# divyanshu-kumar/openh264-wasm

Hardware: AMD Instinct MI355X
Metric: 1080p30 frames/sec encode+decode per GPU (parity vs oracle; OpenH264 parity unpinned) (higher is better)
Workload: dtype u8

## Files before the change

### openh264-wasm_amd/csrc/dec_recon.inc

```
namespace h264mi {

struct DecLaunch { int S, mbw, mbh; const DecDesc *desc; uint32_t *ticket; const DbkDesc *dbk; uint64_t *prof; uint32_t tag; int streamed; };

struct DecGateLaunch { int S; const DecDesc *desc; uint32_t tag; uint32_t rows; };
__global__ __launch_bounds__(64) void dec_gate_kernel(DecGateLaunch a) {
    for (int s = 0; s < a.S; s++) {
        const DecDesc &D = a.desc[s];
        if (!D.st->got_pic) continue;
        GLOBAL uint64_t *prog = gbl(&D.frm->prog);
        WaitClock wc;
        for (unsigned spins = 0; ((spins & 255) != 255) || !wc.expired(); spins++) {
            uint64_t x = 0;
            if (threadIdx.x == 0) x = __hip_atomic_load(prog, __ATOMIC_RELAXED, __HIP_MEMORY_SCOPE_AGENT);
            const uint32_t t = (uint32_t)__builtin_amdgcn_readfirstlane((int)(uint32_t)(x >> 32));
            const uint32_t v = (uint32_t)__builtin_amdgcn_readfirstlane((int)(uint32_t)x);
            if (t == a.tag && v >= a.rows) break;
            __builtin_amdgcn_s_sleep(8);
        }
    }
}

struct DecWaitLaunch { const uint32_t *counter; uint32_t target; uint32_t limit_ticks; };
__global__ __launch_bounds__(64) void dec_wait_counter_kernel(DecWaitLaunch a) {
    const uint64_t t0 = __builtin_amdgcn_s_memrealtime();
// ... 12 lines not shown
    for (unsigned spins = 0;; spins++) {
        uint64_t x = 0;
        if (threadIdx.x == 0) x = __hip_atomic_load(prog, __ATOMIC_RELAXED, __HIP_MEMORY_SCOPE_AGENT);
        const uint32_t t = (uint32_t)__builtin_amdgcn_readfirstlane((int)(uint32_t)(x >> 32));
        const uint32_t v = (uint32_t)__builtin_amdgcn_readfirstlane((int)(uint32_t)x);
        if (t == tag) {
            if (v == H264MI_PROG_ABORT) break;
            if (v >= need) {
                __builtin_amdgcn_fence(__ATOMIC_ACQUIRE, "agent");
                asm volatile("s_waitcnt vmcnt(0)" ::: "memory");
                return true;
            }
        }
        if ((spins & 255) == 255) {
            const int ab = __hip_atomic_load(abort_word, __ATOMIC_RELAXED, __HIP_MEMORY_SCOPE_AGENT);
            if (ab || wc.expired()) break;
        }
        __builtin_amdgcn_s_sleep(2);
    }
    if (threadIdx.x == 0) __hip_atomic_store(abort_word, 1, __ATOMIC_RELAXED, __HIP_MEMORY_SCOPE_AGENT);
    return false;
}

#ifndef H264MI_REC_TILE
#define H264MI_REC_TILE 0
#endif
struct DecLds {
    alignas(16) uint8_t win[4][64 * 64];
    alignas(16) uint8_t winc[2][32 * 32];
    alignas(16) uint32_t cf[208];
#if H264MI_REC_TILE
    alignas(16) uint8_t tile[48 * 48];
#endif
    alignas(16) int16_t res[24][16];
    int dcval[24];
    alignas(16) uint8_t rec[256];
    alignas(16) uint8_t recc[2][64];
#if H264MI_REC_TILE
    alignas(16) uint8_t pcm[384];
#endif
    uint8_t top[24];
    uint8_t topc[2][12];
    uint8_t left[16], leftc[2][8];
    uint8_t n4[16];
    uint32_t gp[3][8];
    uint32_t gm[3][5];
    int8_t modes[16];
    alignas(16) MbInfo info;
    alignas(16) MbInfo linfo;
};

DEV uint32_t dwin4(const DecLds &S, int p, int wr, int gx) {
    const int sl = (gx + 24) & 63;
    const uint32_t *row = (const uint32_t *)&S.win[p][wr * WIN_RING];
    return __builtin_amdgcn_alignbyte(row[((sl >> 2) + 1) & 15], row[sl >> 2], sl & 3);
}

struct TileGet {
    const uint8_t *t; int x0, y0;
    DEV int operator()(int x, int y) const { return t[(y - y0) * 48 + (x - x0)]; }
};
struct GlobGet {
    GLOBAL const uint8_t *p; int w, h;
    DEV int operator()(int x, int y) const { return p[clip3(0, h - 1, y) * w + clip3(0, w - 1, x)]; }
};
template <class G> DEV int g_b1(const G &g, int x, int y) { return tap6(g(x - 2, y), g(x - 1, y), g(x, y), g(x + 1, y), g(x + 2, y), g(x + 3, y)); }
template <class G> DEV int g_b(const G &g, int x, int y) { return clip1((g_b1(g, x, y) + 16) >> 5); }
template <class G> DEV int g_h(const G &g, int x, int y) {
    return clip1((tap6(g(x, y - 2), g(x, y - 1), g(x, y), g(x, y + 1), g(x, y + 2), g(x, y + 3)) + 16) >> 5);
}
template <class G> DEV int g_j(const G &g, int x, int y) {
    return clip1((tap6(g_b1(g, x, y - 2), g_b1(g, x, y - 1), g_b1(g, x, y), g_b1(g, x, y + 1), g_b1(g, x, y + 2), g_b1(g, x, y + 3)) + 512) >> 10);
}
template <class G> DEV int qpel(const G &g, int x, int y, int fx, int fy) {
    switch (fy * 4 + fx) {
    case 0: return g(x, y);
    case 1: return AVG(g(x, y), g_b(g, x, y));
    case 2: return g_b(g, x, y);
    case 3: return AVG(g_b(g, x, y), g(x + 1, y));
    case 4: return AVG(g(x, y), g_h(g, x, y));
    case 5: return AVG(g_b(g, x, y), g_h(g, x, y));
    case 6: return AVG(g_b(g, x, y), g_j(g, x, y));
    case 7: return AVG(g_b(g, x, y), g_h(g, x + 1, y));
    case 8: return g_h(g, x, y);
// ... 148 lines not shown
                    const int dx = I.mv[ras][0], dy = I.mv[ras][1];
                    int mx, my;
                    rmvp(S, mbx, nbm, done, px, py, sw, 0, mx, my);
                    set_part_mv(I, done, px, py, sw, sh, mx + dx, my + dy);
                }
        }
    } else if (type == MI_I4) {
        for (int blk = 0; blk < 16; blk++) S.modes[blk] = I.i4mode[blk];
        const uint32_t top = S.gm[mbx % 3][4] >> 8;
        for (int blk = 0; blk < 16; blk++) {
            const int ras = BLK2RAS[blk], x4 = ras & 3, y4 = ras >> 2;
            const int ma = x4 > 0 ? I.i4mode[ras - 1] : ((nbm & NB_A) ? S.linfo.i4mode[ras + 3] : -1);
            const int mb = y4 > 0 ? I.i4mode[ras - 4] : ((nbm & NB_B) ? (int)((top >> (4 * x4)) & 15) : -1);
            const int pm = (ma < 0 || mb < 0) ? 2 : min(ma, mb);
            const int code = (uint8_t)S.modes[blk];
            I.i4mode[ras] = (int8_t)(code == 0xff ? pm : (code < pm ? code : code + 1));
        }
    }
}

DEV bool mb_in_window(const MbInfo &I) {
    const int b = threadIdx.x & 15;
    const uint32_t mv = ((const uint32_t *)I.mv)[b];
    const int x = (b & 3) * 4 + ((int)(int16_t)(mv & 0xffff) >> 2), y = (b >> 2) * 4 + ((int)(int16_t)(mv >> 16) >> 2);
    const bool ok = min(x, y) >= -24 && max(x, y) + 5 <= 40;
    return __ballot(!ok) == 0;
}

#ifdef H264MI_REC_WPE
#define H264MI_REC_WPE_ATTR __attribute__((amdgpu_waves_per_eu(H264MI_REC_WPE, H264MI_REC_WPE)))
#else
#define H264MI_REC_WPE_ATTR
#endif
__global__ __launch_bounds__(64) H264MI_REC_WPE_ATTR void dec_recon_kernel(DecLaunch a) {
    __shared__ union { DecLds r; DbkLds d; } SH;
    DecLds &S = SH.r;
    __shared__ int s_ticket;
#ifndef H264MI_REC_RELANE
#define H264MI_REC_RELANE 1
#endif
#if H264MI_REC_RELANE
#define lane (e_tid() & 63)
#else
    const int lane = threadIdx.x;
#endif
    if (lane == 0) s_ticket = (int)atomicAdd(a.ticket, 1u);
    wave_lds_sync();
    const int t = uni(s_ticket), nrows = a.S * a.mbh;
    if (t >= nrows) {
// ... 3 lines not shown
        if (DD.active && uni(*DD.active) == 0) return;
        const DbkLaunch dl{a.mbw, a.mbh, a.S, a.dbk, nullptr, nullptr};
        deblock_row(SH.d, dl, DD, dby, DbkSrcGranules{gbl((const uint64_t *)DD.src_gran), a.mbw, dby, (uint32_t)uni((int)*DD.epoch)});
        return;
    }
    const int mby = t / a.S, sidx = t % a.S;
    CONSTANT const DecDesc &D = cst(a.desc)[sidx];
    DecState *st = D.st;
    if (!uni(st->got_pic)) return;
    const uint32_t epoch = (uint32_t)uni((int)st->epoch);
    const int par = uni(st->parity) & 1;
    const bool has_ref = uni(st->has_ref) != 0;
    const Xf XF = xf_consts(lane & 15);
    GLOBAL const uint8_t *R0 = gbl(D.pic[par][0]), *R1 = gbl(D.pic[par][1]), *R2 = gbl(D.pic[par][2]);
    GLOBAL uint32_t *info32 = gbl((uint32_t *)D.info);
    GLOBAL const MbCoef *coefg = gbl((const MbCoef *)D.coef);
    GLOBAL uint64_t *egr = gbl(D.egran);
    int32_t *abort_word = &st->err;
    if (a.streamed && !prog_wait(gbl(&D.frm->prog), a.tag, (uint32_t)mby + 1, abort_word)) return;
    const int mbw = a.mbw, cw = mbw * 16, ch = a.mbh * 16, ccw = cw / 2, cch = ch / 2;
    const int Y = mby * 16;
    GLOBAL uint64_t *grow_prev = gbl(D.gran) + (size_t)(mby > 0 ? mby - 1 : 0) * mbw * H264MI_GRANULES_PER_MB;
    GLOBAL uint64_t *grow = gbl(D.gran) + (size_t)mby * mbw * H264MI_GRANULES_PER_MB;
    const int Y0 = Y - 24;
    GLOBAL const uint8_t *plw[4];
    for (int k = 0; k < 4; k++) plw[k] = gbl((const uint8_t *)D.pl[k]) + (ptrdiff_t)(Y0 + lane) * D.ps;
    GLOBAL const uint8_t *plcw = gbl((const uint8_t *)D.plc[lane >> 5]) + (ptrdiff_t)(mby * 8 - 12 + (lane & 31)) * D.psc;
    uint32_t pf_info = 0, pf_cf[4] = {0, 0, 0, 0};
    u32x4 pf_w[4];
    u32x2 pf_c = {0, 0};
    auto issue = [&](int mx) {
        const int mi = mby * mbw + mx;
        if (lane < 32) pf_info = info32[(size_t)mi * 32 + lane];
        GLOBAL const uint32_t *cf32 = (GLOBAL const uint32_t *)(coefg + mi);
#pragma unroll
        for (int k = 0; k < 4; k++) if (lane + 64 * k < 208) pf_cf[k] = cf32[lane + 64 * k];
        if (has_ref && mx > 0) {
#pragma unroll
            for (int k = 0; k < 4; k++) pf_w[k] = *(GLOBAL const u32x4 *)(plw[k] + 16 * mx + 24);
            pf_c = *(GLOBAL const u32x2 *)(plcw + 8 * mx + 12);
        }
    };
    if (has_ref) {
#pragma unroll
        for (int k = 0; k < 4; k++)
#pragma unroll
            for (int j = 0; j < 4; j++) *(u32x4 *)&S.win[k][lane * WIN_RING + 16 * j] = *(GLOBAL const u32x4 *)(plw[k] - 24 + 16 * j);
#pragma unroll
        for (int j = 0; j < 4; j++) *(u32x2 *)&S.winc[lane >> 5][(lane & 31) * WINC_RING + 8 * j] = *(GLOBAL const u32x2 *)(plcw - 12 + 8 * j);
    }
    issue(0);
    uint64_t t_prev = a.prof ? clock64() : 0, s_prof[9] = {0, 0, 0, 0, 0, 0, 0, 0, 0};
    auto lap = [&](int k) { if (a.prof) { const uint64_t tt = clock64(); s_prof[k] += tt - t_prev; t_prev = tt; } };

    int pix_next = 0;
    for (int mbx = 0; mbx < mbw; mbx++) {
        const int X = mbx * 16, mbi = mby * mbw + mbx;
        if (lane < 32) ((uint32_t *)&S.info)[lane] = pf_info;
        const uint32_t rw0 = __builtin_amdgcn_readfirstlane(pf_info), rw31 = __builtin_amdgcn_readlane(pf_info, 31);
        const int rt = (int)(rw0 & 255);
        {
            if (rt == MI_I16 || rt == MI_IPCM || ((rw0 >> 16) & 255) != 0) {
#pragma unroll
                for (int k = 0; k < 4; k++) if (lane + 64 * k < 208) S.cf[lane + 64 * k] = pf_cf[k];
            }
        }
        if (mbx + 1 < mbw) issue(mbx + 1);
        lap(1);
        if (mby > 0) {
            uint32_t v;
// ... 21 lines not shown
        const uint32_t nbm = uni(mb_nb_mask(mbx, mby, mbw, MB_SLICE_FIRST(rw31)));
        if (rt == MI_PSKIP || rt == MI_P16x16) {
            const uint32_t mvw = resolve_p16_uni(S, mbx, nbm, rt == MI_PSKIP);
            if (lane >= 8 && lane < 13)
                gran_store(grow + (size_t)mbx * H264MI_GRANULES_PER_MB + lane, epoch, lane < 12 ? mvw : (uint32_t)rt | 0x222200u);
            wave_lds_sync();
        } else {
            if (lane == 0) resolve_record(S, mbx, nbm);
            wave_lds_sync();
        }
        if (lane >= 8 && lane < 13 && !(rt == MI_PSKIP || rt == MI_P16x16)) {
            const MbInfo &R = S.info;
            const uint32_t v = lane < 12 ? ((const uint32_t *)R.mv)[12 + lane - 8]
                                         : (uint32_t)R.type | ((uint32_t)(R.i4mode[12] & 15) << 8) | ((uint32_t)(R.i4mode[13] & 15) << 12) |
                                               ((uint32_t)(R.i4mode[14] & 15) << 16) | ((uint32_t)(R.i4mode[15] & 15) << 20);
            gran_store(grow + (size_t)mbx * H264MI_GRANULES_PER_MB + lane, epoch, v);
        }
        if (lane < 32) gran_store(egr + (size_t)mbi * 128 + 96 + lane, epoch, ((const uint32_t *)&S.info)[lane]);
        const MbInfo &I = S.info;
        const int type = I.type;
        const bool intra = type == MI_I4 || type == MI_I16, ipcm = type == MI_IPCM;
        lap(3);
        const MbCoef &CF = *(const MbCoef *)S.cf;
#if H264MI_REC_TILE
        if (ipcm) for (int k = lane; k < 384; k += 64) S.pcm[k] = ((const uint8_t *)&CF)[k];
        const uint8_t *PCM = S.pcm;
#else
        const uint8_t *PCM = (const uint8_t *)&CF;
#endif
        const bool has_top = nbm & NB_B, has_left = nbm & NB_A, has_tr = nbm & NB_C, has_tl = nbm & NB_D;
        const uint32_t *PB = S.gp[mbx % 3], *PC = S.gp[(mbx + 1) % 3], *PD = S.gp[(mbx + 2) % 3];
        if (intra) {
        if (lane < 21) {
            int v = 0;
            if (lane == 0) v = has_tl ? (PD[3] >> 24) & 255 : 0;
            else if (lane <= 16) v = has_top ? (PB[(lane - 1) >> 2] >> (8 * ((lane - 1) & 3))) & 255 : 0;
            else v = has_tr ? (PC[(lane - 17) >> 2] >> (8 * ((lane - 17) & 3))) & 255 : 0;
            S.top[lane] = (uint8_t)v;
        }
        if (lane >= 32 && lane < 50) {
            int pl = (lane - 32) / 9, k = (lane - 32) % 9, v = 0;
            if (k == 0) v = has_tl ? (PD[5 + 2 * pl] >> 24) & 255 : 0;
            else v = has_top ? (PB[4 + 2 * pl + ((k - 1) >> 2)] >> (8 * ((k - 1) & 3))) & 255 : 0;
            S.topc[pl][k] = (uint8_t)v;
        }
        if (!has_left && lane < 16) { S.left[lane] = 0; S.leftc[lane >> 3][lane & 7] = 0; }
        }
        wave_lds_sync();
        lap(4);
        const bool has_res = type != MI_PSKIP && !ipcm;
        if (has_res) {
            const QuantQP ql = make_qqp(I.qp), qcc = make_qqp(I.qpc);
// ... 50 lines not shown
                    }
                    S.n4[lane] = (uint8_t)v;
                }
                wave_lds_sync();
                if (lane < 16) {
                    const int m = I.i4mode[ras];
                    int s4t = S.n4[1] + S.n4[2] + S.n4[3] + S.n4[4], s4l = S.n4[9] + S.n4[10] + S.n4[11] + S.n4[12];
                    int dcv = (bt && bl) ? (s4t + s4l + 4) >> 3 : bl ? (s4l + 2) >> 2 : bt ? (s4t + 2) >> 2 : 128;
                    int pv = m == 2 ? dcv : i4_tap_eval(c_I4.t[m][lane], S.n4);
                    S.rec[(oy + (lane >> 2)) * 16 + ox + (lane & 3)] = (uint8_t)clip1(pv + S.res[ras][lane]);
                }
                wave_lds_sync();
            }
        } else if (type == MI_I16) {
            const I16Ctx k16 = i16_ctx(S, has_top, has_left);
            for (int i = lane; i < 256; i += 64) {
                int x = i & 15, y = i >> 4, ras = (y >> 2) * 4 + (x >> 2);
                S.rec[i] = (uint8_t)clip1(i16_pred(S, k16, I.i16mode, x, y) + S.res[ras][(y & 3) * 4 + (x & 3)]);
            }
        } else if (inwin) {
            {
                const int y = lane >> 2, x0 = (lane & 3) * 4, ras = (y >> 2) * 4 + (x0 >> 2);
                const int mx = I.mv[ras][0], my = I.mv[ras][1];
                const QSel q = qsel((my & 3) * 4 + (mx & 3));
                const int gx = X + x0 + (mx >> 2), wr = Y + y + (my >> 2) - Y0;
                const uint32_t pa = dwin4(S, q.p1, wr + q.dy1, gx + q.dx1), pb = dwin4(S, q.p2, wr + q.dy2, gx + q.dx2);
                const uint32_t pv = (pa | pb) - (((pa ^ pb) & 0xFEFEFEFEu) >> 1);
                uint32_t o = 0;
                if (has_res) {
                    const u32x2 r2 = *(const u32x2 *)&S.res[ras][(y & 3) * 4];
#pragma unroll
                    for (int j = 0; j < 4; j++) {
                        const int rj = (int16_t)(((j < 2 ? r2.x : r2.y) >> (16 * (j & 1))) & 0xffff);
                        o |= (uint32_t)clip1((int)((pv >> (8 * j)) & 255) + rj) << (8 * j);
                    }
                } else o = pv;
                *(uint32_t *)&S.rec[y * 16 + x0] = o;
            }
        } else {
#if H264MI_REC_TILE
            int x0 = 1 << 30, y0 = 1 << 30, x1 = -(1 << 30), y1 = -(1 << 30);
            for (int b = 0; b < 16; b++) {
                int ix = X + (b & 3) * 4 + (I.mv[b][0] >> 2), iy = Y + (b >> 2) * 4 + (I.mv[b][1] >> 2);
                x0 = min(x0, ix - 2); y0 = min(y0, iy - 2); x1 = max(x1, ix + 4 + 3); y1 = max(y1, iy + 4 + 3);
            }
            const bool use_tile = (x1 - x0) <= 48 && (y1 - y0) <= 48;
            if (use_tile) {
                for (int i = lane; i < 48 * 48; i += 64) {
                    int tx = i % 48, ty = i / 48;
                    S.tile[i] = R0[clip3(0, ch - 1, y0 + ty) * cw + clip3(0, cw - 1, x0 + tx)];
                }
                wave_lds_sync();
            }
            const TileGet tg{S.tile, x0, y0};
#endif
            const GlobGet gg{R0, cw, ch};
            for (int i = lane; i < 256; i += 64) {
                int x = i & 15, y = i >> 4, ras = (y >> 2) * 4 + (x >> 2);
                int mx = I.mv[ras][0], my = I.mv[ras][1];
                int gx = X + x + (mx >> 2), gy = Y + y + (my >> 2);
#if H264MI_REC_TILE
                int pv = use_tile ? qpel(tg, gx, gy, mx & 3, my & 3) : qpel(gg, gx, gy, mx & 3, my & 3);
#else
                int pv = qpel(gg, gx, gy, mx & 3, my & 3);
#endif
                S.rec[i] = (uint8_t)clip1(pv + (has_res ? S.res[ras][(y & 3) * 4 + (x & 3)] : 0));
            }
        }
        lap(6);
        if (!ipcm) {
            if (intra) {
                const CCtx kc = chroma_ctx(S, has_top, has_left);
                for (int i = lane; i < 128; i += 64) {
                    int pl = i >> 6, p = i & 63, x = p & 7, y = p >> 3;
                    int dv = chroma_dc_blk(S, kc, pl, x >> 2, y >> 2);
                    int pv = chroma_pred(S, kc, I.cmode, pl, x, y, dv);
                    S.recc[pl][p] = (uint8_t)clip1(pv + S.res[16 + 4 * pl + (y >> 2) * 2 + (x >> 2)][(y & 3) * 4 + (x & 3)]);
                }
            } else if (inwin) {
                const int p = lane, x = p & 7, y = p >> 3, ras = (y >> 1) * 4 + (x >> 1);
                const int mx = I.mv[ras][0], my = I.mv[ras][1], fx = mx & 7, fy = my & 7;
                const int cx = mbx * 8 + x + (mx >> 3), r0 = (y + (my >> 3) + 12) * WINC_RING, r1 = r0 + WINC_RING;
                const int c0 = (cx + 12) & 31, c1 = (cx + 13) & 31;
                const int w00 = (8 - fx) * (8 - fy), w01 = fx * (8 - fy), w10 = (8 - fx) * fy, w11 = fx * fy;
                const int rb = (y >> 2) * 2 + (x >> 2), ri = (y & 3) * 4 + (x & 3);
                int pv[2], rs[2];
#pragma unroll
                for (int pl = 0; pl < 2; pl++) {
// ... 9 lines not shown
                    int ras = (y >> 1) * 4 + (x >> 1);
                    int mx = I.mv[ras][0], my = I.mv[ras][1];
                    int fx = mx & 7, fy = my & 7, gx = mbx * 8 + x + (mx >> 3), gy = mby * 8 + y + (my >> 3);
                    GLOBAL const uint8_t *Rp = pl ? R2 : R1;
                    int xa = clip3(0, ccw - 1, gx), xb = clip3(0, ccw - 1, gx + 1), ya = clip3(0, cch - 1, gy), yb = clip3(0, cch - 1, gy + 1);
                    int A = Rp[ya * ccw + xa], B = Rp[ya * ccw + xb], C = Rp[yb * ccw + xa], E = Rp[yb * ccw + xb];
                    int pv = ((8 - fx) * (8 - fy) * A + fx * (8 - fy) * B + (8 - fx) * fy * C + fx * fy * E + 32) >> 6;
                    S.recc[pl][p] = (uint8_t)clip1(pv + (has_res ? S.res[16 + 4 * pl + (y >> 2) * 2 + (x >> 2)][(y & 3) * 4 + (x & 3)] : 0));
                }
            }
        }
        wave_lds_sync();
        lap(7);
        gran_store(egr + (size_t)mbi * 128 + lane, epoch, ((const uint32_t *)S.rec)[lane]);
        if (lane < 32) gran_store(egr + (size_t)mbi * 128 + 64 + lane, epoch, ((const uint32_t *)S.recc[lane >> 4])[((lane >> 1) & 7) * 2 + (lane & 1)]);
        if (lane < 8) {
            const uint32_t v = lane < 4 ? ((const uint32_t *)S.rec)[60 + lane] : ((const uint32_t *)S.recc[(lane - 4) >> 1])[14 + (lane & 1)];
            gran_store(grow + (size_t)mbx * H264MI_GRANULES_PER_MB + lane, epoch, v);
        }
        if (lane < 16) { S.left[lane] = S.rec[lane * 16 + 15]; S.leftc[lane >> 3][lane & 7] = S.recc[lane >> 3][(lane & 7) * 8 + 7]; }
        if (lane < 32) ((uint32_t *)&S.linfo)[lane] = ((const uint32_t *)&S.info)[lane];
        if (has_ref && mbx + 1 < mbw) {
            const int nx = mbx + 1;
#pragma unroll
            for (int k = 0; k < 4; k++) *(u32x4 *)&S.win[k][lane * WIN_RING + ((16 * nx + 48) & 63)] = pf_w[k];
            *(u32x2 *)&S.winc[lane >> 5][(lane & 31) * WINC_RING + ((8 * nx + 24) & 31)] = pf_c;
        }
        wave_lds_sync();
        lap(8);
    }
    if (a.prof && lane == 0) {
#pragma unroll
        for (int k = 1; k < 9; k++) atomicAdd((unsigned long long *)&a.prof[k], (unsigned long long)s_prof[k]);
    }
#if H264MI_REC_RELANE
#undef lane
#endif
}

struct DecEndLaunch { int S; const DecDesc *desc; int check; };
__global__ void dec_end_kernel(DecEndLaunch a) {
    int s = blockIdx.x * blockDim.x + threadIdx.x;
    if (s >= a.S) return;
    if (a.check) dec_frame_check(a.desc[s]);
    DecState *st = a.desc[s].st;
    if (st->got_pic) {
        st->outpar = st->parity ^ 1;
        if (!st->nonref) { st->parity ^= 1; st->has_ref = 1; }
// ... 32 lines not shown
```

### openh264-wasm_amd/csrc/enc_planes.inc

```
namespace h264mi {

struct PlanesLaunch { int S, cw, ch; const PlanesDesc *pd; int ystrips; };

constexpr int PT_H = 16, PT_Q = 256;
static_assert((2 * H264MI_LPADY) % PT_H == 0, "planes strips tile the padded height");
DEV uint32_t planes_row_bytes(const uint8_t *row, int x, int cw) {
    const uint32_t v = *(const uint32_t *)(row + clip3(0, cw - 4, x));
    return x < 0 ? (v & 255u) * 0x01010101u : (x >= cw ? (v >> 24) * 0x01010101u : v);
}
DEV void ref_planes_chroma(const PlanesLaunch &a, const PlanesDesc &D, int i);
DEV void ref_planes_block(const PlanesLaunch &a, int bx, int by, int bz, int gx) {
    const PlanesDesc &D = a.pd[bz];
    if (D.active && *D.active == 0) return;
    if (by >= a.ystrips) {
        ref_planes_chroma(a, D, ((by - a.ystrips) * gx + bx) * PT_Q + (int)threadIdx.x);
        return;
    }
    const int cw = a.cw, ch = a.ch;
    const int pw = cw + 2 * H264MI_LPADX;
    const int q = bx * PT_Q + (int)threadIdx.x;
    if (q * 4 >= pw) return;
    const int x0 = q * 4 - H264MI_LPADX;
    const int ya = by * PT_H - H264MI_LPADY;
    const uint8_t *ref = D.src[D.parity ? (*D.parity & 1) : 0][0];
// ... 25 lines not shown
    for (int r = 0; r < PT_H; r++) {
        absorb(5);
        if (r + 1 < PT_H) issue(r + 6);
        uint32_t vb = 0, vh = 0, vj = 0;
#pragma unroll
        for (int k = 0; k < 4; k++) {
            const int sh = 8 * k;
            const int Hv = tap6((Mw[0] >> sh) & 255, (Mw[1] >> sh) & 255, (Mw[2] >> sh) & 255, (Mw[3] >> sh) & 255,
                                (Mw[4] >> sh) & 255, (Mw[5] >> sh) & 255);
            const int J = tap6(b1(0, k), b1(1, k), b1(2, k), b1(3, k), b1(4, k), b1(5, k));
            vb |= (uint32_t)clip1_shr(b1(2, k) + 16, 5) << sh;
            vh |= (uint32_t)clip1_shr(Hv + 16, 5) << sh;
            vj |= (uint32_t)clip1_shr(J + 512, 10) << sh;
        }
        const ptrdiff_t o = (ptrdiff_t)(ya + r) * D.ps + x0;
        *(uint32_t *)(pG + o) = Mw[2];
        *(uint32_t *)(pB + o) = vb;
        *(uint32_t *)(pH + o) = vh;
        *(uint32_t *)(pJ + o) = vj;
#pragma unroll
        for (int i = 0; i < 5; i++) { Mw[i] = Mw[i + 1]; Bw[i][0] = Bw[i + 1][0]; Bw[i][1] = Bw[i + 1][1]; }
    }
}
__global__ __launch_bounds__(PT_Q, 8) void ref_planes_kernel(PlanesLaunch a) {
    ref_planes_block(a, blockIdx.x, blockIdx.y, blockIdx.z, gridDim.x);
}

DEV void ref_planes_chroma(const PlanesLaunch &a, const PlanesDesc &D, int i) {
    const int cwc = a.cw / 2, chc = a.ch / 2;
    const int pw = cwc + 2 * H264MI_CPADX, ph = chc + 2 * H264MI_CPADY, q = pw / 4, strips = (ph + PT_H - 1) / PT_H;
    const int pl = i / (q * strips);
    if (pl >= 2) return;
    i -= pl * q * strips;
    const int st = i / q, xx = (i - st * q) * 4, x = xx - H264MI_CPADX;
    static_assert(H264MI_CPADX % 4 == 0, "chroma quads are dword-aligned");
    const uint8_t *base = D.src[D.parity ? (*D.parity & 1) : 0][1 + pl];
#pragma unroll 1
    for (int r = 0; r < PT_H; r++) {
        const int yy = st * PT_H + r;
        if (yy >= ph) break;
        const int y = yy - H264MI_CPADY;
        *(uint32_t *)(D.plc[pl] + (ptrdiff_t)y * D.psc + x) = planes_row_bytes(base + (size_t)clip3(0, chc - 1, y) * cwc, x, cwc);
    }
}

static void ref_planes_grid(int cw, int ch, int &gx, int &gy, int &ystrips) {
    const int quads = (cw + 2 * H264MI_LPADX) / 4;
    gx = (quads + PT_Q - 1) / PT_Q;
    ystrips = (ch + 2 * H264MI_LPADY + PT_H - 1) / PT_H;
    const int cq = 2 * ((cw / 2 + 2 * H264MI_CPADX) / 4) * ((ch / 2 + 2 * H264MI_CPADY + PT_H - 1) / PT_H);
    gy = ystrips + (cq + gx * PT_Q - 1) / (gx * PT_Q);
}
static int launch_ref_planes(int S, int cw, int ch, const PlanesDesc *pd, hipStream_t st) {
    int gx, gy, ystrips;
    ref_planes_grid(cw, ch, gx, gy, ystrips);
    const PlanesLaunch pla{S, cw, ch, pd, ystrips};
    hipLaunchKernelGGL(ref_planes_kernel, dim3(gx, gy, S), dim3(PT_Q), 0, st, pla);
    return hipGetLastError() == hipSuccess ? 0 : -1;
}

static_assert(PACK_THREADS == PT_Q, "enc_post_kernel: one block size");
struct PostLaunch { PackLaunch pk; PlanesLaunch pl; int gx, gy; };
__global__ __launch_bounds__(PT_Q) void enc_post_kernel(PostLaunch a) {
    const int b = (int)blockIdx.x;
    if (b < a.pk.S) { enc_pack_block(a.pk, b); return; }
    const int r = b - a.pk.S, per = a.gx * a.gy, z = r / per, yx = r - z * per, y = yx / a.gx;
    ref_planes_block(a.pl, yx - y * a.gx, y, z, a.gx);
}
__global__ __launch_bounds__(PT_Q) void enc_post_slices_kernel(PostLaunch a) {
    const int b = (int)blockIdx.x;
    if (b < a.pk.S) { enc_pack_block_slices(a.pk, b); return; }
    const int r = b - a.pk.S, per = a.gx * a.gy, z = r / per, yx = r - z * per, y = yx / a.gx;
    ref_planes_block(a.pl, yx - y * a.gx, y, z, a.gx);
}
static int launch_enc_post(const PackLaunch &pk, int cw, int ch, const PlanesDesc *pd, hipStream_t st, bool slices) {
    int gx, gy, ystrips;
    ref_planes_grid(cw, ch, gx, gy, ystrips);
    const PostLaunch pl{pk, PlanesLaunch{pk.S, cw, ch, pd, ystrips}, gx, gy};
    if (slices) hipLaunchKernelGGL(enc_post_slices_kernel, dim3(pk.S + gx * gy * pk.S), dim3(PT_Q), 0, st, pl);
    else hipLaunchKernelGGL(enc_post_kernel, dim3(pk.S + gx * gy * pk.S), dim3(PT_Q), 0, st, pl);
// ... 5 lines not shown
```

### openh264-wasm_amd/csrc/h264mi_types.h

```cpp
#pragma once
#include <stdint.h>

#define H264MI_MAX_STREAMS 256
#define H264MI_MB_SLOT_DWORDS 640
#define H264MI_ENC_MAX_MBW 512
#define H264MI_GRANULES_PER_MB 16
#define H264MI_DBK_GRANULES_PER_MB 24
#define H264MI_LPADX 40
#define H264MI_LPADY 32
#define H264MI_CPADX 20
#define H264MI_CPADY 16

enum { MI_I4 = 0, MI_I16 = 1, MI_P16x16 = 2, MI_PSKIP = 3, MI_P16x8 = 4, MI_P8x16 = 5, MI_P8x8 = 6, MI_IPCM = 7 };

struct MbInfo {
    uint8_t type, qp, cbp, i16mode;
    uint8_t cmode, qpc, pad0, pad1;
    int8_t i4mode[16];
    int8_t ref[4];
    uint8_t nnz[24];
    int16_t mvd[2];
    uint8_t sub[4];
    int16_t mv[16][2];
    int32_t pad2;
// ... 132 lines not shown
    NalEnt e[H264MI_MAX_NALS];
    SliceEnt sl[H264MI_MAX_SLICES];
    uint64_t prog;
    uint32_t sdone, pad_p;
};
#define H264MI_PROG_ABORT 0xFFFFFFFFu
#define MB_SLICE_FIRST(w) ((int)((w) & 0xFFFFFu))
#define MB_SLICE_IDC(w) ((int)(((w) >> 20) & 3u))
#define MB_SLICE_OFFA(w) (2 * (((int)((w) << 6)) >> 28))
#define MB_SLICE_OFFB(w) (2 * (((int)((w) << 2)) >> 28))
struct DecInput { const uint8_t *nal; const int32_t *size_dev; int32_t size, fmt; uint8_t *out; int32_t *got; };

struct DecDesc {
    uint8_t *cur[3];
    uint8_t *pic[2][3];
    MbInfo *info;
    MbCoef *coef;
    uint64_t *gran;
    uint64_t *dgran;
    DecState *st;
    DecFrame *frm;
    int32_t cw, ch;
    uint64_t *egran;
    uint8_t *pl[4];
    uint8_t *plc[2];
    int32_t ps, psc;
};
```

### openh264-wasm_amd/csrc/runtime_dec.inc

```
namespace h264mi {

constexpr int DEC_PSTREAMS = 3;
struct DecCtx {
    int mbw, mbh, nmb, cw, ch, S, B;
    int NG;
    hipStream_t stream;
    bool own_stream;
    static constexpr int PMAX = 16;
    int np = DEC_PSTREAMS;
    hipStream_t pst[PMAX] = {};
    int cu_lo = 0, cu_hi = 0;
    std::vector<hipEvent_t> ev_hdr, ev_parsed, ev_recon;
    hipEvent_t ev_in = nullptr;
    int grp = 0;
    uint32_t calls = 0;
    uint8_t *d_pool = nullptr;
    size_t pool_bytes = 0;
    DecState *d_st = nullptr;
    DecDesc *d_desc = nullptr;
    DbkDesc *d_dbk = nullptr;
    PlanesDesc *d_pd = nullptr;
    DecInput *d_in = nullptr;
    uint32_t *d_ticket = nullptr;
    std::vector<DecDesc> h_desc;
// ... 80 lines not shown
    (void)hipFree(c->d_prof);
    (void)hipFree(c->d_rprof);
    if (c->own_stream) (void)hipStreamDestroy(c->stream);
    delete c;
}

static DecCtx *dec_create(int mbw, int mbh, int S, hipStream_t stream, int B = 1, int ng = 0, int np = DEC_PSTREAMS) {
    if (mbw <= 0 || mbh <= 0 || mbw > H264MI_MAX_MBS || mbh > H264MI_MAX_MBS || S <= 0 || B <= 0 ||
        S > H264MI_MAX_STREAMS || S * B > 4096 || ng > 16 || np < 1 || np > DecCtx::PMAX) return nullptr;
    wait_limit_from_env();
    DecCtx *c = new DecCtx();
    c->mbw = mbw; c->mbh = mbh; c->nmb = mbw * mbh; c->cw = mbw * 16; c->ch = mbh * 16; c->S = S; c->B = B;
    c->NG = ng > 0 ? std::max(2, ng) : std::max(2, std::min(16, 32 / B));
    c->np = np;
    if (stream) { c->stream = stream; c->own_stream = false; }
    else { if (hipStreamCreateWithFlags(&c->stream, hipStreamNonBlocking) != hipSuccess) { delete c; return nullptr; } c->own_stream = true; }
    const size_t ysz = (size_t)c->cw * c->ch, csz = ysz / 4, pic = ysz + 2 * csz;
    auto al = [](size_t x) { return (x + 255) & ~(size_t)255; };
    const size_t off_p0 = al(pic), off_p1 = off_p0 + al(pic), off_gran = off_p1 + al(pic);
    const size_t off_dgran = off_gran + al(8 * (size_t)H264MI_GRANULES_PER_MB * c->nmb);
    const size_t off_egr = off_dgran + al(8 * (size_t)H264MI_DBK_GRANULES_PER_MB * c->nmb);
    const size_t lps = (size_t)c->cw + 2 * H264MI_LPADX, lph = (size_t)c->ch + 2 * H264MI_LPADY;
    const size_t cps = (size_t)c->cw / 2 + 2 * H264MI_CPADX, cph = (size_t)c->ch / 2 + 2 * H264MI_CPADY;
    const size_t off_pl = off_egr + al(8 * 128 * (size_t)c->nmb), off_plc = off_pl + 4 * al(lps * lph);
    const size_t per_stream = off_plc + 2 * al(cps * cph);
    const size_t off_coef = al(sizeof(MbInfo) * c->nmb), off_frm = off_coef + al(sizeof(MbCoef) * c->nmb);
    const size_t per_slot = off_frm + al(sizeof(DecFrame));
    const int NS = c->NG * B;
    const size_t nsl = (size_t)S * NS;
    const size_t hdr = al(sizeof(DecState) * S) + al(sizeof(PlanesDesc) * S) + al(sizeof(DecDesc) * nsl) + al(sizeof(DbkDesc) * nsl) +
                       al(sizeof(DecInput) * nsl) + al(sizeof(uint32_t) * 2 * NS);
    const size_t total = hdr + per_stream * S + per_slot * nsl;
    if (hipMalloc(&c->d_pool, total) != hipSuccess) { if (c->own_stream) (void)hipStreamDestroy(c->stream); delete c; return nullptr; }
    c->pool_bytes = total;
    (void)hipMemsetAsync(c->d_pool, 0, total, c->stream);
    uint8_t *p = c->d_pool;
    c->d_st = (DecState *)p; p += al(sizeof(DecState) * S);
    c->d_pd = (PlanesDesc *)p; p += al(sizeof(PlanesDesc) * S);
    c->d_desc = (DecDesc *)p; p += al(sizeof(DecDesc) * nsl);
    c->d_dbk = (DbkDesc *)p; p += al(sizeof(DbkDesc) * nsl);
    c->d_in = (DecInput *)p; p += al(sizeof(DecInput) * nsl);
    c->d_ticket = (uint32_t *)p; p += al(sizeof(uint32_t) * 2 * NS);
    uint8_t *streams = p, *slots = p + per_stream * S;
    c->h_desc.resize(nsl);
    if (hipHostMalloc((void **)&c->h_in, sizeof(DecInput) * nsl, hipHostMallocDefault) != hipSuccess) c->h_in = nullptr;
    std::vector<DbkDesc> hd(nsl);
    std::vector<PlanesDesc> hp(S);
    for (int f = 0; f < NS; f++)
        for (int s = 0; s < S; s++) {
            uint8_t *b = streams + per_stream * s, *q = slots + per_slot * ((size_t)f * S + s);
            DecDesc &d = c->h_desc[(size_t)f * S + s];
            uint8_t *cur = b, *p0 = b + off_p0, *p1 = b + off_p1;
            d.cur[0] = cur; d.cur[1] = cur + ysz; d.cur[2] = cur + ysz + csz;
            d.pic[0][0] = p0; d.pic[0][1] = p0 + ysz; d.pic[0][2] = p0 + ysz + csz;
            d.pic[1][0] = p1; d.pic[1][1] = p1 + ysz; d.pic[1][2] = p1 + ysz + csz;
            d.gran = (uint64_t *)(b + off_gran); d.dgran = (uint64_t *)(b + off_dgran);
            d.info = (MbInfo *)q; d.coef = (MbCoef *)(q + off_coef); d.frm = (DecFrame *)(q + off_frm);
            d.st = c->d_st + s; d.cw = c->cw; d.ch = c->ch; d.egran = (uint64_t *)(b + off_egr);
            for (int k = 0; k < 4; k++) d.pl[k] = b + off_pl + k * al(lps * lph) + H264MI_LPADY * lps + H264MI_LPADX;
            for (int k = 0; k < 2; k++) d.plc[k] = b + off_plc + k * al(cps * cph) + H264MI_CPADY * cps + H264MI_CPADX;
            d.ps = (int)lps; d.psc = (int)cps;
            if (f == 0) {
                PlanesDesc &pd = hp[s];
                for (int i = 0; i < 3; i++) { pd.src[0][i] = d.pic[0][i]; pd.src[1][i] = d.pic[1][i]; }
                pd.parity = &c->d_st[s].parity; pd.active = &c->d_st[s].got_pic;
                for (int k = 0; k < 4; k++) pd.pl[k] = d.pl[k];
                pd.plc[0] = d.plc[0]; pd.plc[1] = d.plc[1]; pd.ps = d.ps; pd.psc = d.psc;
            }
            DbkDesc &k = hd[(size_t)f * S + s];
            for (int i = 0; i < 3; i++) { k.rec[i] = d.cur[i]; k.out[0][i] = d.pic[1][i]; k.out[1][i] = d.pic[0][i]; }
            k.info = d.info; k.dgran = d.dgran; k.epoch = &c->d_st[s].epoch; k.disable = nullptr;
            k.active = &c->d_st[s].got_pic; k.parity = &c->d_st[s].parity; k.abort_word = &c->d_st[s].err; k.src_gran = d.egran;
        }
    (void)hipMemcpyAsync(c->d_desc, c->h_desc.data(), sizeof(DecDesc) * nsl, hipMemcpyHostToDevice, c->stream);
    (void)hipMemcpyAsync(c->d_dbk, hd.data(), sizeof(DbkDesc) * nsl, hipMemcpyHostToDevice, c->stream);
    (void)hipMemcpyAsync(c->d_pd, hp.data(), sizeof(PlanesDesc) * S, hipMemcpyHostToDevice, c->stream);
    if (getenv("H264MI_RECON_PROF") && hipMalloc(&c->d_rprof, sizeof(uint64_t) * 16) == hipSuccess)
        (void)hipMemsetAsync(c->d_rprof, 0, sizeof(uint64_t) * 16, c->stream);
    if (getenv("H264MI_PARSE_PROF") && hipMalloc(&c->d_prof, sizeof(uint64_t) * 16 * nsl) == hipSuccess)
        (void)hipMemsetAsync(c->d_prof, 0, sizeof(uint64_t) * 16 * nsl, c->stream);
    c->lds_bytes = RING_BYTES + 2 * 4 * (size_t)mbw;
    c->lds_min = c->lds_bytes;
    bool ok = c->h_in && hipEventCreateWithFlags(&c->ev_in, hipEventDisableTiming) == hipSuccess;
    for (int i = 0; i < c->np && ok; i++) ok = hipStreamCreateWithFlags(&c->pst[i], hipStreamNonBlocking) == hipSuccess;
    for (auto *v : {&c->ev_hdr, &c->ev_parsed, &c->ev_recon}) {
        v->assign(c->NG, nullptr);
        for (int g = 0; g < c->NG && ok; g++) ok = hipEventCreateWithFlags(&(*v)[g], hipEventDisableTiming) == hipSuccess;
    }
    for (int g = 0; g < c->NG && ok; g++) ok = hipEventRecord(c->ev_recon[g], c->stream) == hipSuccess && hipEventRecord(c->ev_hdr[g], c->stream) == hipSuccess;
// ... 41 lines not shown
    for (int f = 0; f < n; f++) {
        const DecDesc *df = dd + (size_t)f * S;
        hipLaunchKernelGGL(dec_frame_begin_kernel, dim3((S + 63) / 64), dim3(64), 0, c->stream,
                           DecBeginLaunch{S, f, dd, streamed, c->d_ticket + 2 * (slot0 + f)});
        if (streamed && f == 0 && c->gate_rows > 0)
            hipLaunchKernelGGL(dec_gate_kernel, dim3(1), dim3(64), 0, c->stream, DecGateLaunch{S, df, tag, (uint32_t)c->gate_rows});
        if (rg_counter && f < rg_count)
            hipLaunchKernelGGL(dec_wait_counter_kernel, dim3(1), dim3(64), 0, c->stream,
                               DecWaitLaunch{rg_counter, rg_target + (uint32_t)f * rg_step, rg_limit});
        if (dec_time_mark(c, 0, c->stream)) return -1;
        hipLaunchKernelGGL(dec_recon_kernel, dim3(2 * S * c->mbh), dim3(64), 0, c->stream,
                           DecLaunch{S, c->mbw, c->mbh, df, c->d_ticket + 2 * (slot0 + f), c->d_dbk + (size_t)(slot0 + f) * S, c->d_rprof,
                                     tag, streamed});
        if (dec_time_mark(c, 0, c->stream)) return -1;
        if (streamed && f == 0) HIPCHECK(hipStreamWaitEvent(c->stream, c->ev_parsed[g], 0));
        hipLaunchKernelGGL(dec_end_kernel, dim3((S + 63) / 64), dim3(64), 0, c->stream, DecEndLaunch{S, df, streamed});
        if (outputs && in[0].fmt == H264MI_FMT_RGBA) {
            const dim3 cg = color_grid(c->cw, c->ch, S);
            hipLaunchKernelGGL(dec_output_rgba_kernel, dim3(cg.x, S), dim3(256), 0, c->stream,
                               DecOutLaunch{S, c->cw, c->ch, df, c->d_in + (size_t)(slot0 + f) * S});
        } else if (outputs)
            hipLaunchKernelGGL(dec_output_kernel, dim3((2 * c->ch + 3) / 4, S), dim3(256), 0, c->stream,
                               DecOutLaunch{S, c->cw, c->ch, df, c->d_in + (size_t)(slot0 + f) * S});
        if (launch_ref_planes(S, c->cw, c->ch, c->d_pd, c->stream) != 0) return -1;
    }
    HIPCHECK(hipEventRecord(c->ev_recon[g], c->stream));
    HIPCHECK(hipGetLastError());
    c->grp = (g + 1) % c->NG;
    c->calls++;
    return 0;
}
static std::vector<uint32_t> cu_mask(int lo, int hi, bool complement) {
    int ncu = 0, dev = 0;
    if (hipGetDevice(&dev) != hipSuccess || hipDeviceGetAttribute(&ncu, hipDeviceAttributeMultiprocessorCount, dev) != hipSuccess || ncu <= 0)
        ncu = 256;
    std::vector<uint32_t> m((size_t)(ncu + 31) / 32, 0);
    for (int i = 0; i < ncu; i++)
        if ((i >= lo && i < hi) != complement) m[(size_t)i / 32] |= 1u << (i % 32);
    return m;
}
static int dec_set_parse_cus(DecCtx *c, int lo, int hi) {
    if (lo < 0 || hi < lo) return -1;
    if (dec_sync_all(c) != hipSuccess) return -1;
    const std::vector<uint32_t> m = cu_mask(lo, hi, false);
    c->cu_lo = lo; c->cu_hi = hi;
    c->lds_bytes = lo == hi ? c->lds_min : std::max(c->lds_min, (size_t)40 * 1024);
    for (int i = 0; i < DecCtx::PMAX; i++) {
// ... 35 lines not shown
```

Baseline: 4840.

## Interpolate decoder luma subpel on the fly from a single padded reference plane

The decoder previously precomputed four half-pel luma planes (full, b, h, j) per reference and kept four LDS windows. Now only the integer-pel plane is padded and stored. The recon kernel computes the b/h/j 6-tap filters from a single LDS window, using wave ballots so each filter runs only when some lane needs it. This cuts plane-generation bandwidth, global prefetch traffic and LDS footprint, at the cost of extra ALU work per inter macroblock. The window bounds check now accounts for the filter taps and for chroma.

```diff
diff --git a/openh264-wasm_amd/csrc/dec_recon.inc b/openh264-wasm_amd/csrc/dec_recon.inc
--- a/openh264-wasm_amd/csrc/dec_recon.inc
+++ b/openh264-wasm_amd/csrc/dec_recon.inc
@@ -58,23 +58,17 @@
     return false;
 }
 
-#ifndef H264MI_REC_TILE
-#define H264MI_REC_TILE 0
-#endif
+constexpr int DWIN_ROWS = 64;
+constexpr int DWIN_LO = -24, DWIN_HI = 40;
+constexpr int DWINC_LO = -12, DWINC_HI = 20;
 struct DecLds {
-    alignas(16) uint8_t win[4][64 * 64];
+    alignas(16) uint8_t win[DWIN_ROWS * WIN_RING];
     alignas(16) uint8_t winc[2][32 * 32];
     alignas(16) uint32_t cf[208];
-#if H264MI_REC_TILE
-    alignas(16) uint8_t tile[48 * 48];
-#endif
     alignas(16) int16_t res[24][16];
     int dcval[24];
     alignas(16) uint8_t rec[256];
     alignas(16) uint8_t recc[2][64];
-#if H264MI_REC_TILE
-    alignas(16) uint8_t pcm[384];
-#endif
     uint8_t top[24];
     uint8_t topc[2][12];
     uint8_t left[16], leftc[2][8];
@@ -86,16 +80,77 @@
     alignas(16) MbInfo linfo;
 };
 
-DEV uint32_t dwin4(const DecLds &S, int p, int wr, int gx) {
+DEV uint32_t dwin4(const DecLds &S, int wr, int gx) {
     const int sl = (gx + 24) & 63;
-    const uint32_t *row = (const uint32_t *)&S.win[p][wr * WIN_RING];
+    const uint32_t *row = (const uint32_t *)&S.win[wr * WIN_RING];
     return __builtin_amdgcn_alignbyte(row[((sl >> 2) + 1) & 15], row[sl >> 2], sl & 3);
 }
 
-struct TileGet {
-    const uint8_t *t; int x0, y0;
-    DEV int operator()(int x, int y) const { return t[(y - y0) * 48 + (x - x0)]; }
-};
+struct WRow { uint32_t lo, mid, hi; };
+DEV WRow dwin_row(const DecLds &S, int wr, int gx) {
+    const int sl = (gx - 2 + 24) & 63, d = sl >> 2, sh = sl & 3;
+    const uint32_t *row = (const uint32_t *)&S.win[clip3(0, DWIN_ROWS - 1, wr) * WIN_RING];
+    const uint32_t d0 = row[d], d1 = row[(d + 1) & 15], d2 = row[(d + 2) & 15];
+    return WRow{__builtin_amdgcn_alignbyte(d1, d0, sh), __builtin_amdgcn_alignbyte(d2, d1, sh), (d2 >> (8 * sh)) & 255u};
+}
+DEV uint32_t wrow_quad(const WRow &r, int dx) { return __builtin_amdgcn_alignbyte(r.mid, r.lo, 2 + dx); }
+DEV void wrow_b1(const WRow &r, int t[4]) {
+    int s[9];
+#pragma unroll
+    for (int k = 0; k < 4; k++) { s[k] = (r.lo >> (8 * k)) & 255; s[4 + k] = (r.mid >> (8 * k)) & 255; }
+    s[8] = r.hi;
+#pragma unroll
+    for (int k = 0; k < 4; k++) t[k] = tap6(s[k], s[k + 1], s[k + 2], s[k + 3], s[k + 4], s[k + 5]);
+}
+DEV uint32_t pack_clip_shr(const int t[4], int rnd, int sh) {
+    uint32_t o = 0;
+#pragma unroll
+    for (int k = 0; k < 4; k++) o |= (uint32_t)clip1_shr(t[k] + rnd, sh) << (8 * k);
+    return o;
+}
+DEV uint32_t dec_luma_frac(const DecLds &S, int wr, int gx, int idx) {
+    const QSel q = qsel(idx);
+    const bool ub = __ballot(q.p1 == 1 || q.p2 == 1) != 0, uh = __ballot(q.p1 == 2 || q.p2 == 2) != 0;
+    const bool uj = __ballot(q.p1 == 3 || q.p2 == 3) != 0;
+    const int gdx = q.p1 == 0 ? q.dx1 : q.dx2, gdy = q.p1 == 0 ? q.dy1 : q.dy2;
+    const int bdy = q.p1 == 1 ? q.dy1 : q.dy2, hdx = q.p1 == 2 ? q.dx1 : q.dx2;
+    const WRow r2 = dwin_row(S, wr, gx);
+    WRow r3 = r2;
+    uint32_t vb = 0, vh = 0, vj = 0;
+    if (uh || uj) {
+        const WRow r0 = dwin_row(S, wr - 2, gx), r1 = dwin_row(S, wr - 1, gx), r4 = dwin_row(S, wr + 2, gx), r5 = dwin_row(S, wr + 3, gx);
+        r3 = dwin_row(S, wr + 1, gx);
+        if (uh) {
+            const uint32_t c0 = wrow_quad(r0, hdx), c1 = wrow_quad(r1, hdx), c2 = wrow_quad(r2, hdx), c3 = wrow_quad(r3, hdx);
+            const uint32_t c4 = wrow_quad(r4, hdx), c5 = wrow_quad(r5, hdx);
+            int t[4];
+#pragma unroll
+            for (int k = 0; k < 4; k++) {
+                const int s = 8 * k;
+                t[k] = tap6((c0 >> s) & 255, (c1 >> s) & 255, (c2 >> s) & 255, (c3 >> s) & 255, (c4 >> s) & 255, (c5 >> s) & 255);
+            }
+            vh = pack_clip_shr(t, 16, 5);
+        }
+        if (uj) {
+            int t0[4], t1[4], t2[4], t3[4], t4[4], t5[4], t[4];
+            wrow_b1(r0, t0); wrow_b1(r1, t1); wrow_b1(r2, t2); wrow_b1(r3, t3); wrow_b1(r4, t4); wrow_b1(r5, t5);
+#pragma unroll
+            for (int k = 0; k < 4; k++) t[k] = tap6(t0[k], t1[k], t2[k], t3[k], t4[k], t5[k]);
+            vj = pack_clip_shr(t, 512, 10);
+        }
+    }
+    if (ub) {
+        const WRow rb{bdy ? r3.lo : r2.lo, bdy ? r3.mid : r2.mid, bdy ? r3.hi : r2.hi};
+        int t[4];
+        wrow_b1(rb, t);
+        vb = pack_clip_shr(t, 16, 5);
+    }
+    const uint32_t vg = gdy ? wrow_quad(r3, 0) : wrow_quad(r2, gdx);
+    const uint32_t pa = q.p1 == 0 ? vg : (q.p1 == 1 ? vb : (q.p1 == 2 ? vh : vj));
+    const uint32_t pb = q.p2 == 0 ? vg : (q.p2 == 1 ? vb : (q.p2 == 2 ? vh : vj));
+    return (pa | pb) - (((pa ^ pb) & 0xFEFEFEFEu) >> 1);
+}
+
 struct GlobGet {
     GLOBAL const uint8_t *p; int w, h;
     DEV int operator()(int x, int y) const { return p[clip3(0, h - 1, y) * w + clip3(0, w - 1, x)]; }
@@ -290,9 +345,13 @@
 DEV bool mb_in_window(const MbInfo &I) {
     const int b = threadIdx.x & 15;
     const uint32_t mv = ((const uint32_t *)I.mv)[b];
-    const int x = (b & 3) * 4 + ((int)(int16_t)(mv & 0xffff) >> 2), y = (b >> 2) * 4 + ((int)(int16_t)(mv >> 16) >> 2);
-    const bool ok = min(x, y) >= -24 && max(x, y) + 5 <= 40;
-    return __ballot(!ok) == 0;
+    const int mvx = (int16_t)(mv & 0xffff), mvy = (int16_t)(mv >> 16);
+    const int x = (b & 3) * 4 + (mvx >> 2), y = (b >> 2) * 4 + (mvy >> 2);
+    const int fx = (mvx & 3) != 0, fy = (mvy & 3) != 0;
+    const int cx = (b & 3) * 2 + (mvx >> 3), cy = (b >> 2) * 2 + (mvy >> 3);
+    const bool okl = min(x - 2 * fx, y - 2 * fy) >= DWIN_LO && max(x + 3 * fx, y + 3 * fy) + 3 < DWIN_HI;
+    const bool okc = min(cx, cy) >= DWINC_LO && max(cx, cy) + 2 < DWINC_HI;
+    return __ballot(!(okl && okc)) == 0;
 }
 
 #ifdef H264MI_REC_WPE
@@ -342,12 +401,14 @@
     const int Y = mby * 16;
     GLOBAL uint64_t *grow_prev = gbl(D.gran) + (size_t)(mby > 0 ? mby - 1 : 0) * mbw * H264MI_GRANULES_PER_MB;
     GLOBAL uint64_t *grow = gbl(D.gran) + (size_t)mby * mbw * H264MI_GRANULES_PER_MB;
-    const int Y0 = Y - 24;
-    GLOBAL const uint8_t *plw[4];
-    for (int k = 0; k < 4; k++) plw[k] = gbl((const uint8_t *)D.pl[k]) + (ptrdiff_t)(Y0 + lane) * D.ps;
+    const int Y0 = Y + DWIN_LO;
+    static_assert(DWIN_HI - DWIN_LO == DWIN_ROWS && DWIN_ROWS == 64 && WIN_RING == 64, "one window row per lane, 64-column ring");
+    static_assert(-DWIN_LO <= H264MI_LPADY && DWIN_HI - 16 <= H264MI_LPADY && -DWIN_LO <= H264MI_LPADX && DWIN_HI - 16 <= H264MI_LPADX,
+                  "the window of an edge macroblock lies inside the plane's padding");
+    GLOBAL const uint8_t *plw = gbl((const uint8_t *)D.pl) + (ptrdiff_t)(Y0 + lane) * D.ps;
     GLOBAL const uint8_t *plcw = gbl((const uint8_t *)D.plc[lane >> 5]) + (ptrdiff_t)(mby * 8 - 12 + (lane & 31)) * D.psc;
     uint32_t pf_info = 0, pf_cf[4] = {0, 0, 0, 0};
-    u32x4 pf_w[4];
+    u32x4 pf_w = {0, 0, 0, 0};
     u32x2 pf_c = {0, 0};
     auto issue = [&](int mx) {
         const int mi = mby * mbw + mx;
@@ -356,16 +417,13 @@
 #pragma unroll
         for (int k = 0; k < 4; k++) if (lane + 64 * k < 208) pf_cf[k] = cf32[lane + 64 * k];
         if (has_ref && mx > 0) {
-#pragma unroll
-            for (int k = 0; k < 4; k++) pf_w[k] = *(GLOBAL const u32x4 *)(plw[k] + 16 * mx + 24);
+            pf_w = *(GLOBAL const u32x4 *)(plw + 16 * mx + 24);
             pf_c = *(GLOBAL const u32x2 *)(plcw + 8 * mx + 12);
         }
     };
     if (has_ref) {
 #pragma unroll
-        for (int k = 0; k < 4; k++)
-#pragma unroll
-            for (int j = 0; j < 4; j++) *(u32x4 *)&S.win[k][lane * WIN_RING + 16 * j] = *(GLOBAL const u32x4 *)(plw[k] - 24 + 16 * j);
+        for (int j = 0; j < 4; j++) *(u32x4 *)&S.win[lane * WIN_RING + 16 * j] = *(GLOBAL const u32x4 *)(plw - 24 + 16 * j);
 #pragma unroll
         for (int j = 0; j < 4; j++) *(u32x2 *)&S.winc[lane >> 5][(lane & 31) * WINC_RING + 8 * j] = *(GLOBAL const u32x2 *)(plcw - 12 + 8 * j);
     }
@@ -433,12 +491,7 @@
         const bool intra = type == MI_I4 || type == MI_I16, ipcm = type == MI_IPCM;
         lap(3);
         const MbCoef &CF = *(const MbCoef *)S.cf;
-#if H264MI_REC_TILE
-        if (ipcm) for (int k = lane; k < 384; k += 64) S.pcm[k] = ((const uint8_t *)&CF)[k];
-        const uint8_t *PCM = S.pcm;
-#else
         const uint8_t *PCM = (const uint8_t *)&CF;
-#endif
         const bool has_top = nbm & NB_B, has_left = nbm & NB_A, has_tr = nbm & NB_C, has_tl = nbm & NB_D;
         const uint32_t *PB = S.gp[mbx % 3], *PC = S.gp[(mbx + 1) % 3], *PD = S.gp[(mbx + 2) % 3];
         if (intra) {
@@ -535,10 +588,11 @@
             {
                 const int y = lane >> 2, x0 = (lane & 3) * 4, ras = (y >> 2) * 4 + (x0 >> 2);
                 const int mx = I.mv[ras][0], my = I.mv[ras][1];
-                const QSel q = qsel((my & 3) * 4 + (mx & 3));
+                const int idx = (my & 3) * 4 + (mx & 3);
                 const int gx = X + x0 + (mx >> 2), wr = Y + y + (my >> 2) - Y0;
-                const uint32_t pa = dwin4(S, q.p1, wr + q.dy1, gx + q.dx1), pb = dwin4(S, q.p2, wr + q.dy2, gx + q.dx2);
-                const uint32_t pv = (pa | pb) - (((pa ^ pb) & 0xFEFEFEFEu) >> 1);
+                uint32_t pv;
+                if (__ballot(idx != 0) == 0) pv = dwin4(S, wr, gx);
+                else pv = dec_luma_frac(S, wr, gx, idx);
                 uint32_t o = 0;
                 if (has_res) {
                     const u32x2 r2 = *(const u32x2 *)&S.res[ras][(y & 3) * 4];
@@ -551,32 +605,12 @@
                 *(uint32_t *)&S.rec[y * 16 + x0] = o;
             }
         } else {
-#if H264MI_REC_TILE
-            int x0 = 1 << 30, y0 = 1 << 30, x1 = -(1 << 30), y1 = -(1 << 30);
-            for (int b = 0; b < 16; b++) {
-                int ix = X + (b & 3) * 4 + (I.mv[b][0] >> 2), iy = Y + (b >> 2) * 4 + (I.mv[b][1] >> 2);
-                x0 = min(x0, ix - 2); y0 = min(y0, iy - 2); x1 = max(x1, ix + 4 + 3); y1 = max(y1, iy + 4 + 3);
-            }
-            const bool use_tile = (x1 - x0) <= 48 && (y1 - y0) <= 48;
-            if (use_tile) {
-                for (int i = lane; i < 48 * 48; i += 64) {
-                    int tx = i % 48, ty = i / 48;
-                    S.tile[i] = R0[clip3(0, ch - 1, y0 + ty) * cw + clip3(0, cw - 1, x0 + tx)];
-                }
-                wave_lds_sync();
-            }
-            const TileGet tg{S.tile, x0, y0};
-#endif
             const GlobGet gg{R0, cw, ch};
             for (int i = lane; i < 256; i += 64) {
                 int x = i & 15, y = i >> 4, ras = (y >> 2) * 4 + (x >> 2);
                 int mx = I.mv[ras][0], my = I.mv[ras][1];
                 int gx = X + x + (mx >> 2), gy = Y + y + (my >> 2);
-#if H264MI_REC_TILE
-                int pv = use_tile ? qpel(tg, gx, gy, mx & 3, my & 3) : qpel(gg, gx, gy, mx & 3, my & 3);
-#else
                 int pv = qpel(gg, gx, gy, mx & 3, my & 3);
-#endif
                 S.rec[i] = (uint8_t)clip1(pv + (has_res ? S.res[ras][(y & 3) * 4 + (x & 3)] : 0));
             }
         }
@@ -632,8 +666,7 @@
         if (lane < 32) ((uint32_t *)&S.linfo)[lane] = ((const uint32_t *)&S.info)[lane];
         if (has_ref && mbx + 1 < mbw) {
             const int nx = mbx + 1;
-#pragma unroll
-            for (int k = 0; k < 4; k++) *(u32x4 *)&S.win[k][lane * WIN_RING + ((16 * nx + 48) & 63)] = pf_w[k];
+            *(u32x4 *)&S.win[lane * WIN_RING + ((16 * nx + 48) & 63)] = pf_w;
             *(u32x2 *)&S.winc[lane >> 5][(lane & 31) * WINC_RING + ((8 * nx + 24) & 31)] = pf_c;
         }
         wave_lds_sync();
diff --git a/openh264-wasm_amd/csrc/enc_planes.inc b/openh264-wasm_amd/csrc/enc_planes.inc
--- a/openh264-wasm_amd/csrc/enc_planes.inc
+++ b/openh264-wasm_amd/csrc/enc_planes.inc
@@ -71,9 +71,6 @@
         for (int i = 0; i < 5; i++) { Mw[i] = Mw[i + 1]; Bw[i][0] = Bw[i + 1][0]; Bw[i][1] = Bw[i + 1][1]; }
     }
 }
-__global__ __launch_bounds__(PT_Q, 8) void ref_planes_kernel(PlanesLaunch a) {
-    ref_planes_block(a, blockIdx.x, blockIdx.y, blockIdx.z, gridDim.x);
-}
 
 DEV void ref_planes_chroma(const PlanesLaunch &a, const PlanesDesc &D, int i) {
     const int cwc = a.cw / 2, chc = a.ch / 2;
@@ -100,11 +97,29 @@
     const int cq = 2 * ((cw / 2 + 2 * H264MI_CPADX) / 4) * ((ch / 2 + 2 * H264MI_CPADY + PT_H - 1) / PT_H);
     gy = ystrips + (cq + gx * PT_Q - 1) / (gx * PT_Q);
 }
-static int launch_ref_planes(int S, int cw, int ch, const PlanesDesc *pd, hipStream_t st) {
+__global__ __launch_bounds__(PT_Q) void dec_planes_kernel(PlanesLaunch a) {
+    const PlanesDesc &D = a.pd[blockIdx.z];
+    if (D.active && *D.active == 0) return;
+    if ((int)blockIdx.y >= a.ystrips) {
+        ref_planes_chroma(a, D, (((int)blockIdx.y - a.ystrips) * (int)gridDim.x + (int)blockIdx.x) * PT_Q + (int)threadIdx.x);
+        return;
+    }
+    const int cw = a.cw, ch = a.ch;
+    const int q = (int)blockIdx.x * PT_Q + (int)threadIdx.x;
+    if (q * 4 >= cw + 2 * H264MI_LPADX) return;
+    const int x0 = q * 4 - H264MI_LPADX, ya = (int)blockIdx.y * PT_H - H264MI_LPADY;
+    const uint8_t *ref = D.src[D.parity ? (*D.parity & 1) : 0][0];
+    uint32_t v[PT_H];
+#pragma unroll
+    for (int r = 0; r < PT_H; r++) v[r] = planes_row_bytes(ref + (size_t)clip3(0, ch - 1, ya + r) * cw, x0, cw);
+#pragma unroll
+    for (int r = 0; r < PT_H; r++) *(uint32_t *)(D.pl[0] + (ptrdiff_t)(ya + r) * D.ps + x0) = v[r];
+}
+static int launch_dec_planes(int S, int cw, int ch, const PlanesDesc *pd, hipStream_t st) {
     int gx, gy, ystrips;
     ref_planes_grid(cw, ch, gx, gy, ystrips);
     const PlanesLaunch pla{S, cw, ch, pd, ystrips};
-    hipLaunchKernelGGL(ref_planes_kernel, dim3(gx, gy, S), dim3(PT_Q), 0, st, pla);
+    hipLaunchKernelGGL(dec_planes_kernel, dim3(gx, gy, S), dim3(PT_Q), 0, st, pla);
     return hipGetLastError() == hipSuccess ? 0 : -1;
 }
 
diff --git a/openh264-wasm_amd/csrc/h264mi_types.h b/openh264-wasm_amd/csrc/h264mi_types.h
--- a/openh264-wasm_amd/csrc/h264mi_types.h
+++ b/openh264-wasm_amd/csrc/h264mi_types.h
@@ -178,7 +178,7 @@
     DecFrame *frm;
     int32_t cw, ch;
     uint64_t *egran;
-    uint8_t *pl[4];
+    uint8_t *pl;
     uint8_t *plc[2];
     int32_t ps, psc;
 };
diff --git a/openh264-wasm_amd/csrc/runtime_dec.inc b/openh264-wasm_amd/csrc/runtime_dec.inc
--- a/openh264-wasm_amd/csrc/runtime_dec.inc
+++ b/openh264-wasm_amd/csrc/runtime_dec.inc
@@ -126,7 +126,7 @@
     const size_t off_egr = off_dgran + al(8 * (size_t)H264MI_DBK_GRANULES_PER_MB * c->nmb);
     const size_t lps = (size_t)c->cw + 2 * H264MI_LPADX, lph = (size_t)c->ch + 2 * H264MI_LPADY;
     const size_t cps = (size_t)c->cw / 2 + 2 * H264MI_CPADX, cph = (size_t)c->ch / 2 + 2 * H264MI_CPADY;
-    const size_t off_pl = off_egr + al(8 * 128 * (size_t)c->nmb), off_plc = off_pl + 4 * al(lps * lph);
+    const size_t off_pl = off_egr + al(8 * 128 * (size_t)c->nmb), off_plc = off_pl + al(lps * lph);
     const size_t per_stream = off_plc + 2 * al(cps * cph);
     const size_t off_coef = al(sizeof(MbInfo) * c->nmb), off_frm = off_coef + al(sizeof(MbCoef) * c->nmb);
     const size_t per_slot = off_frm + al(sizeof(DecFrame));
@@ -161,14 +161,14 @@
             d.gran = (uint64_t *)(b + off_gran); d.dgran = (uint64_t *)(b + off_dgran);
             d.info = (MbInfo *)q; d.coef = (MbCoef *)(q + off_coef); d.frm = (DecFrame *)(q + off_frm);
             d.st = c->d_st + s; d.cw = c->cw; d.ch = c->ch; d.egran = (uint64_t *)(b + off_egr);
-            for (int k = 0; k < 4; k++) d.pl[k] = b + off_pl + k * al(lps * lph) + H264MI_LPADY * lps + H264MI_LPADX;
+            d.pl = b + off_pl + H264MI_LPADY * lps + H264MI_LPADX;
             for (int k = 0; k < 2; k++) d.plc[k] = b + off_plc + k * al(cps * cph) + H264MI_CPADY * cps + H264MI_CPADX;
             d.ps = (int)lps; d.psc = (int)cps;
             if (f == 0) {
                 PlanesDesc &pd = hp[s];
                 for (int i = 0; i < 3; i++) { pd.src[0][i] = d.pic[0][i]; pd.src[1][i] = d.pic[1][i]; }
                 pd.parity = &c->d_st[s].parity; pd.active = &c->d_st[s].got_pic;
-                for (int k = 0; k < 4; k++) pd.pl[k] = d.pl[k];
+                pd.pl[0] = d.pl; pd.pl[1] = pd.pl[2] = pd.pl[3] = nullptr;
                 pd.plc[0] = d.plc[0]; pd.plc[1] = d.plc[1]; pd.ps = d.ps; pd.psc = d.psc;
             }
             DbkDesc &k = hd[(size_t)f * S + s];
@@ -256,7 +256,7 @@
         } else if (outputs)
             hipLaunchKernelGGL(dec_output_kernel, dim3((2 * c->ch + 3) / 4, S), dim3(256), 0, c->stream,
                                DecOutLaunch{S, c->cw, c->ch, df, c->d_in + (size_t)(slot0 + f) * S});
-        if (launch_ref_planes(S, c->cw, c->ch, c->d_pd, c->stream) != 0) return -1;
+        if (launch_dec_planes(S, c->cw, c->ch, c->d_pd, c->stream) != 0) return -1;
     }
     HIPCHECK(hipEventRecord(c->ev_recon[g], c->stream));
     HIPCHECK(hipGetLastError());
```

After: 5591 (median of 6 runs). 1.16x the previous value.
